# toufique-morshed/CPU-GPU-TFHE

Measured on AMD Instinct MI355X. Metric: gate bootstraps/sec (bootsNAND, N=1024), higher is better.
Workload: dtype f64 (FFT external product; Torus32 in/out, rounded products exact)

## Files before the change

cpu-gpu-tfhe_amd/csrc/keyswitch.hip:

```cpp
#include "engine.h"
#include "modarith.h"

#include <algorithm>
#include <cstdlib>

namespace tfhe_amd {

namespace {


constexpr int kKs4Cols = 4;
constexpr int kKs4Blocks = 126;
constexpr int kKs4I = 32;
#ifndef TFHE_AMD_KS4_THREADS
#define TFHE_AMD_KS4_THREADS 256
#endif
constexpr int kKs4Threads = TFHE_AMD_KS4_THREADS;
constexpr int kKs4ChunkU4 = kKs4I * kKsT * 3;
static_assert(kKs4ChunkU4 % kKs4Threads == 0, "chunk must split evenly");
constexpr int kKs4Pieces = kKs4ChunkU4 / kKs4Threads;

struct KsLane {
    const int32_t *ua, *ua2;
    uint32_t b;
    int32_t *ra, *rb;
};
struct KsPlain {
    const int32_t *u_a, *u_b, *u2_a, *u2_b;
    int32_t add_b;
    int32_t *res_a, *res_b;
    int B;
    __device__ int count() const { return B; }
    __device__ KsLane lane(int ct) const {
        KsLane l;
        l.ua = u_a + (size_t)ct * kN;
        l.ua2 = u2_a ? u2_a + (size_t)ct * kN : nullptr;
        l.b = (uint32_t)u_b[ct] + (uint32_t)add_b + (u2_b ? (uint32_t)u2_b[ct] : 0u);
        l.ra = res_a + (size_t)ct * kn;
        l.rb = res_b + ct;
        return l;
    }
};
struct KsRows {
    const CircKs *ks;
    const int32_t *u_a, *u_b;
    int32_t *wa, *wb;
    int B, nks;
    __device__ int count() const { return B * nks; }
    __device__ KsLane lane(int ct) const {
        const int g = ct / B, k = ct - g * B;
        const CircKs e = ks[g];
        const size_t s1 = (size_t)e.r1 * B + k, so = (size_t)e.out * B + k;
        KsLane l;
        l.ua = u_a + s1 * kN;
        l.b = (uint32_t)u_b[s1] + (uint32_t)e.add_b;
        l.ua2 = nullptr;
        if (e.r2 >= 0) {
            const size_t s2 = (size_t)e.r2 * B + k;
            l.ua2 = u_a + s2 * kN;
            l.b += (uint32_t)u_b[s2];
        }
        l.ra = wa + so * kn;
        l.rb = wb + so;
        return l;
    }
};

template <class P, int SPLIT>
__global__ __launch_bounds__(kKs4Threads) void k_keyswitch_v4(const uint4 *__restrict__ ksk4, P io) {
    __shared__ __attribute__((aligned(16))) uint4 buf[2][kKs4I * kKsT * 4];
    const int part = SPLIT > 1 ? (int)(blockIdx.x % SPLIT) : 0;
    const int bid = SPLIT > 1 ? (int)(blockIdx.x / SPLIT) : (int)blockIdx.x;
    const int xcd = bid & 7, k = bid >> 3;
    const int cb = (k & 15) * 8 + xcd;
    const int ctg = k >> 4;
    if (cb >= kKs4Blocks) return;
    const int tid = threadIdx.x;
    const int ct = ctg * kKs4Threads + tid;
    const bool valid = ct < io.count();
    const KsLane ln = io.lane(valid ? ct : 0);
    for (int t = tid; t < 2 * kKs4I * kKsT; t += kKs4Threads) buf[t >> 8][(t & 255) * 4] = make_uint4(0, 0, 0, 0);

    uint32_t acc[kKs4Cols];
#pragma unroll
    for (int c = 0; c < kKs4Cols; ++c) acc[c] = 0;
    if (SPLIT == 1 && cb * kKs4Cols <= kn && kn < cb * kKs4Cols + kKs4Cols) acc[kn - cb * kKs4Cols] = ln.b;
    constexpr int kIPart = kN / SPLIT;
    const int ibeg = part * kIPart;

    const uint4 *src = ksk4 + ((size_t)cb * kN + ibeg) * kKsT * 3 + tid;
    const uint4 *pa = reinterpret_cast<const uint4 *>(ln.ua + ibeg);
    const uint4 *pa2 = ln.ua2 ? reinterpret_cast<const uint4 *>(ln.ua2 + ibeg) : nullptr;
    int dst[kKs4Pieces];
    uint4 p[kKs4Pieces];
#pragma unroll
    for (int l = 0; l < kKs4Pieces; ++l) {
        const int t = tid + kKs4Threads * l;
        dst[l] = (t / 3) * 4 + (t - 3 * (t / 3)) + 1;
    }
#pragma unroll
    for (int l = 0; l < kKs4Pieces; ++l) p[l] = src[kKs4Threads * l];
    uint4 av[kKs4I / 4], av2[kKs4I / 4];
#pragma unroll
    for (int v = 0; v < kKs4I / 4; ++v) {
        av[v] = pa[v];
        av2[v] = pa2 ? pa2[v] : make_uint4(0, 0, 0, 0);
    }
#pragma unroll
    for (int l = 0; l < kKs4Pieces; ++l) buf[0][dst[l]] = p[l];
    __syncthreads();
    for (int i0 = 0, b = 0; i0 < kIPart; i0 += kKs4I, b ^= 1) {
        uint32_t a[kKs4I];
#pragma unroll
        for (int v = 0; v < kKs4I / 4; ++v) {
            a[4 * v] = av[v].x + av2[v].x + kKsPrecOffset;
            a[4 * v + 1] = av[v].y + av2[v].y + kKsPrecOffset;
            a[4 * v + 2] = av[v].z + av2[v].z + kKsPrecOffset;
            a[4 * v + 3] = av[v].w + av2[v].w + kKsPrecOffset;
        }
        const bool more = i0 + kKs4I < kIPart;
        if (more) {
            const uint4 *sn = src + (size_t)(i0 + kKs4I) * kKsT * 3;
#pragma unroll
            for (int l = 0; l < kKs4Pieces; ++l) p[l] = sn[kKs4Threads * l];
#pragma unroll
            for (int v = 0; v < kKs4I / 4; ++v) {
                av[v] = pa[(i0 + kKs4I) / 4 + v];
                if (pa2) av2[v] = pa2[(i0 + kKs4I) / 4 + v];
            }
        }
        const uint4 *cur = buf[b];
#pragma unroll
        for (int ii = 0; ii < kKs4I; ++ii) {
            const uint32_t ab = a[ii];
#pragma unroll
            for (int j = 0; j < kKsT; ++j) {
                const uint32_t aij = (ab >> (32 - (j + 1) * kKsBasebit)) & (kKsBase - 1);
                const uint4 r = cur[(ii * kKsT + j) * 4 + (int)aij];
                acc[0] -= r.x; acc[1] -= r.y; acc[2] -= r.z; acc[3] -= r.w;
            }
            asm volatile("" : "+v"(acc[0]), "+v"(acc[1]), "+v"(acc[2]), "+v"(acc[3]));
        }
        if (more) {
            uint4 *nb = buf[b ^ 1];
#pragma unroll
            for (int l = 0; l < kKs4Pieces; ++l) nb[dst[l]] = p[l];
        }
        __syncthreads();
    }
    if (!valid) return;
#pragma unroll
    for (int c = 0; c < kKs4Cols; ++c) {
        const int col = cb * kKs4Cols + c;
        int32_t *dst = col < kn ? ln.ra + col : col == kn ? ln.rb : nullptr;
        if (!dst) continue;
        if (SPLIT > 1) atomicAdd(reinterpret_cast<unsigned int *>(dst), acc[c]);
        else *dst = (int32_t)acc[c];
    }
}

constexpr int kKsSmallChunks = 64;
constexpr int kKsSmallI = kN / kKsSmallChunks;

template <class P>
__global__ __launch_bounds__(512) void k_keyswitch_small_init(P io) {
    const KsLane ln = io.lane(blockIdx.x);
    const int col = threadIdx.x;
    if (col < kn) ln.ra[col] = 0;
    else if (col == kn) *ln.rb = (int32_t)ln.b;
}

#ifndef TFHE_AMD_KS_SMALL_U
#define TFHE_AMD_KS_SMALL_U 2
#endif
constexpr int kKsSmallU = TFHE_AMD_KS_SMALL_U;
template <class P, int U>
__global__ __launch_bounds__(512) void k_keyswitch_small(const int32_t *__restrict__ ksk, P io) {
    const int chunk = blockIdx.x, col = threadIdx.x;
    const KsLane ln = io.lane(blockIdx.y);
    if (col > kn) return;
    const int i0 = chunk * kKsSmallI;
    uint32_t acc = 0;
#pragma unroll U
    for (int ii = 0; ii < kKsSmallI; ++ii) {
        const int i = i0 + ii;
        const uint32_t ab = (uint32_t)ln.ua[i] + (ln.ua2 ? (uint32_t)ln.ua2[i] : 0u) + kKsPrecOffset;
        const int32_t *row = ksk + (size_t)i * kKsT * 3 * kKsRow + col;
#pragma unroll
        for (int j = 0; j < kKsT; ++j) {
            const uint32_t h = (ab >> (32 - (j + 1) * kKsBasebit)) & (kKsBase - 1);
            const uint32_t v = (uint32_t)row[(j * 3 + (int)(h ? h : 1u) - 1) * kKsRow];
            acc -= h ? v : 0u;
        }
    }
    int32_t *dst = col < kn ? ln.ra + col : ln.rb;
    atomicAdd(reinterpret_cast<unsigned int *>(dst), acc);
}

typedef int ks5_v4i __attribute__((ext_vector_type(4)));
typedef int ks5_v16i __attribute__((ext_vector_type(16)));
#ifndef TFHE_AMD_KS5_WAVES
#define TFHE_AMD_KS5_WAVES 8
#endif
constexpr int kKs5Waves = TFHE_AMD_KS5_WAVES;
constexpr int kKs5Threads = 64 * kKs5Waves;
constexpr int kKs5Ch = 16;
constexpr int kKs5Nb = 64;
constexpr int kKs5Cols = 8 * kKs5Nb;
static_assert(kKs5Cols > kn, "the N-blocks cover every column and b");
constexpr int kKs5ChU4 = kKs5Ch * 64;
static_assert(kKs5ChU4 % kKs5Threads == 0, "chunk must split evenly");
constexpr int kKs5Pieces = kKs5ChU4 / kKs5Threads;
#ifndef TFHE_AMD_KS5_G
#define TFHE_AMD_KS5_G 8
#endif
constexpr int kKs5G = TFHE_AMD_KS5_G;

template <class P, int SPLIT, int MS>
__global__ __launch_bounds__(kKs5Threads) void k_keyswitch_v5(const uint4 *__restrict__ w5, P io) {
    constexpr int kM = 32 * kKs5Waves * MS;
    constexpr int kG = kKs5G / MS;
    static_assert(kKs5Ch % kG == 0, "groups split the chunk");
    __shared__ __attribute__((aligned(16))) uint2 lut[16][32];
    __shared__ __attribute__((aligned(16))) uint4 bs[2][kKs5Ch][64];
    __shared__ __attribute__((aligned(16))) uint8_t dg[2][2][kM][kKs5Ch];
    const int bid = (int)blockIdx.x, xcd = bid & 7, kk = bid >> 3;
    const int nb = xcd + 8 * (kk & 7), part = (kk >> 3) % SPLIT, mt = (kk >> 3) / SPLIT;
    constexpr int kChunks = kN / kKs5Ch / SPLIT;
    const int c0 = part * kChunks;
    const int tid = threadIdx.x, wave = tid >> 6, l = tid & 63, r = l & 31, hh = l >> 5;
    for (int e = tid; e < 16 * 32; e += kKs5Threads)
        lut[e >> 5][e & 31] = make_uint2(1u << (8 * ((e >> 7) & 3)), 1u << (8 * ((e >> 5) & 3)));
    constexpr int kPer = kKs5Ch * MS / 2;
    constexpr int kU4 = kPer / 4;
    static_assert(kKs5Threads * kPer == kM * kKs5Ch, "loader mapping");
    const int lct = (tid * MS) >> 1, lpart = MS == 1 ? (tid & 1) : 0;
    const int lg = mt * kM + lct;
    const KsLane lln = io.lane(lg < io.count() ? lg : 0);
    const uint4 *pa = reinterpret_cast<const uint4 *>(lln.ua) + kU4 * lpart;
    const uint4 *pa2 = reinterpret_cast<const uint4 *>(lln.ua2 ? lln.ua2 : lln.ua) + kU4 * lpart;
    const uint32_t m2 = lln.ua2 ? 0xffffffffu : 0u;
    pa += c0 * (kKs5Ch / 4);
    pa2 += c0 * (kKs5Ch / 4);
    uint4 uu[kU4], vv[kU4];
#pragma unroll
    for (int q = 0; q < kU4; ++q) {
        uu[q] = pa[q];
        vv[q] = pa2[q];
    }
    auto put_digits = [&](int buf) {
        uint32_t hi[kPer / 4], lo[kPer / 4];
#pragma unroll
        for (int q = 0; q < kU4; ++q) {
            const uint32_t w[4] = {uu[q].x + (vv[q].x & m2) + kKsPrecOffset, uu[q].y + (vv[q].y & m2) + kKsPrecOffset,
                                   uu[q].z + (vv[q].z & m2) + kKsPrecOffset, uu[q].w + (vv[q].w & m2) + kKsPrecOffset};
            hi[q] = (w[0] >> 24) | ((w[1] >> 24) << 8) | ((w[2] >> 24) << 16) | ((w[3] >> 24) << 24);
            lo[q] = ((w[0] >> 16) & 255u) | (((w[1] >> 16) & 255u) << 8) | (((w[2] >> 16) & 255u) << 16) |
                    (((w[3] >> 16) & 255u) << 24);
        }
        if (kU4 == 2) {
            *reinterpret_cast<uint2 *>(&dg[buf][0][lct][kPer * lpart]) = make_uint2(hi[0], hi[1]);
            *reinterpret_cast<uint2 *>(&dg[buf][1][lct][kPer * lpart]) = make_uint2(lo[0], lo[1]);
        } else {
            *reinterpret_cast<uint4 *>(&dg[buf][0][lct][0]) = make_uint4(hi[0], hi[1], hi[2 % kU4], hi[3 % kU4]);
            *reinterpret_cast<uint4 *>(&dg[buf][1][lct][0]) = make_uint4(lo[0], lo[1], lo[2 % kU4], lo[3 % kU4]);
        }
    };
    const uint4 *src = w5 + ((size_t)nb * kN + (size_t)c0 * kKs5Ch) * 64 + tid;
    uint4 p[kKs5Pieces];
#pragma unroll
    for (int q = 0; q < kKs5Pieces; ++q) p[q] = src[q * kKs5Threads];
#pragma unroll
    for (int q = 0; q < kKs5Pieces; ++q) (&bs[0][0][0])[tid + q * kKs5Threads] = p[q];
    put_digits(0);
    __syncthreads();
    ks5_v16i acc[MS];
#pragma unroll
    for (int m = 0; m < MS; ++m) acc[m] = ks5_v16i{};
    for (int c = 0; c < kChunks; ++c) {
        const bool more = c + 1 < kChunks;
        {
            const int cn = more ? c + 1 : c;
            const uint4 *sn = src + (size_t)cn * kKs5ChU4;
#pragma unroll
            for (int q = 0; q < kKs5Pieces; ++q) p[q] = sn[q * kKs5Threads];
#pragma unroll
            for (int q = 0; q < kU4; ++q) {
                uu[q] = pa[cn * (kKs5Ch / 4) + q];
                vv[q] = pa2[cn * (kKs5Ch / 4) + q];
            }
        }
        uint32_t xw[MS][4];
#pragma unroll
        for (int m = 0; m < MS; ++m) {
            const uint4 xd = *reinterpret_cast<const uint4 *>(&dg[c & 1][hh][wave * 32 * MS + 32 * m + r][0]);
            xw[m][0] = xd.x; xw[m][1] = xd.y; xw[m][2] = xd.z; xw[m][3] = xd.w;
        }
        const uint4(*cur)[64] = bs[c & 1];
#pragma unroll
        for (int g = 0; g < kKs5Ch; g += kG) {
            uint4 av[MS][kG], bv[kG];
#pragma unroll
            for (int q = 0; q < kG; ++q) {
                const int ii = g + q;
#pragma unroll
                for (int m = 0; m < MS; ++m) {
                    const uint32_t xb = xw[m][ii >> 2] >> (8 * (ii & 3));
                    const uint2 d01 = lut[(xb >> 4) & 15u][r], d23 = lut[xb & 15u][r];
                    av[m][q] = make_uint4(d01.x, d01.y, d23.x, d23.y);
                }
                bv[q] = cur[ii][l];
            }
            __builtin_amdgcn_sched_barrier(0);
#pragma unroll
            for (int q = 0; q < kG; ++q) {
                const ks5_v4i b = {(int)bv[q].x, (int)bv[q].y, (int)bv[q].z, (int)bv[q].w};
#pragma unroll
                for (int m = 0; m < MS; ++m) {
                    const ks5_v4i a = {(int)av[m][q].x, (int)av[m][q].y, (int)av[m][q].z, (int)av[m][q].w};
                    acc[m] = __builtin_amdgcn_mfma_i32_32x32x32_i8(a, b, acc[m], 0, 0, 0);
                }
            }
        }
        if (more) {
#pragma unroll
            for (int q = 0; q < kKs5Pieces; ++q) (&bs[(c + 1) & 1][0][0])[tid + q * kKs5Threads] = p[q];
            put_digits((c + 1) & 1);
        }
        __syncthreads();
    }
    const int col = nb * 8 + (r >> 2);
    const uint32_t lsh = 8u * (uint32_t)(l & 3);
#pragma unroll
    for (int m = 0; m < MS; ++m) {
#pragma unroll
        for (int reg = 0; reg < 16; ++reg) {
            uint32_t v = (uint32_t)acc[m][reg] << lsh;
            v += (uint32_t)__shfl_xor((int)v, 1, 64);
            v += (uint32_t)__shfl_xor((int)v, 2, 64);
            const int ctm = mt * kM + wave * 32 * MS + 32 * m + (reg & 3) + 8 * (reg >> 2) + 4 * hh;
            if ((l & 3) == 0 && ctm < io.count() && col <= kn) {
                const KsLane lm = io.lane(ctm);
                if (SPLIT > 1) atomicAdd(reinterpret_cast<unsigned int *>(col < kn ? lm.ra + col : lm.rb), 0u - v);
                else if (col < kn) lm.ra[col] = (int32_t)(0u - v);
                else *lm.rb = (int32_t)(lm.b - v);
            }
        }
    }
}

__global__ __launch_bounds__(256) void k_ksk_to_v5(const int32_t *__restrict__ ksk, uint4 *__restrict__ w5) {
    const size_t total = (size_t)kKs5Nb * kN * 64;
    for (size_t t = (size_t)blockIdx.x * 256 + threadIdx.x; t < total; t += (size_t)gridDim.x * 256) {
        const int l = (int)(t & 63);
        const int i = (int)((t >> 6) % kN);
        const int nb = (int)(t / ((size_t)kN * 64));
        const int col = nb * 8 + ((l & 31) >> 2), limb = l & 3, h = l >> 5;
        uint32_t w[4];
#pragma unroll
        for (int tt = 0; tt < 4; ++tt) {
            uint32_t word = 0;
            for (int hh = 1; hh < 4; ++hh) {
                if (col > kn) break;
                uint32_t v = (uint32_t)ksk[(((size_t)i * kKsT + 4 * h + tt) * 3 + (hh - 1)) * kKsRow + col];
                int8_t sb = 0;
                for (int b = 0; b <= limb; ++b) {
                    sb = (int8_t)(v & 0xffu);
                    v = (v - (uint32_t)(int32_t)sb) >> 8;
                }
                word |= (uint32_t)(uint8_t)sb << (8 * hh);
            }
            w[tt] = word;
        }
        w5[t] = make_uint4(w[0], w[1], w[2], w[3]);
    }
}

__global__ __launch_bounds__(256) void k_ksk_to_v4(const int32_t *__restrict__ ksk, uint4 *__restrict__ ksk4) {
    const size_t pieces = (size_t)kKs4Blocks * kN * kKsT * 3;
    for (size_t t = (size_t)blockIdx.x * 256 + threadIdx.x; t < pieces; t += (size_t)gridDim.x * 256) {
        const int cb = (int)(t / ((size_t)kN * kKsT * 3));
        const size_t row = t % ((size_t)kN * kKsT * 3);
        ksk4[t] = *reinterpret_cast<const uint4 *>(ksk + row * kKsRow + cb * kKs4Cols);
    }
}

}

static int ks_split_max() { return 768; }
bool ks5_enabled() {
    static const bool v = [] {
        const char *e = getenv("TFHE_AMD_KS5");
        return !(e && atoi(e) == 0);
    }();
    return v;
}
static int ks5_split(int mtiles) {
    int sp = 1;
    while (sp < 8 && mtiles * kKs5Nb * sp < 512) sp *= 2;
    return sp;
}
template <class P, int MS>
static void launch_ks5(const uint4 *w5, int count, const P &io, hipStream_t s) {
    const int mtiles = (count + 32 * kKs5Waves * MS - 1) / (32 * kKs5Waves * MS);
    const int split = ks5_split(mtiles);
    if (split > 1) hipLaunchKernelGGL(k_keyswitch_small_init<P>, dim3(count), dim3(512), 0, s, io);
    const dim3 grid(mtiles * kKs5Nb * split);
    trace_kernel(split == 8 ? "k_keyswitch_v5(int8-mfma+split8)" : split == 4 ? "k_keyswitch_v5(int8-mfma+split4)"
                 : split == 2 ? "k_keyswitch_v5(int8-mfma+split2)" : "k_keyswitch_v5(int8-mfma)");
    switch (split) {
    case 8: hipLaunchKernelGGL((k_keyswitch_v5<P, 8, MS>), grid, dim3(kKs5Threads), 0, s, w5, io); break;
    case 4: hipLaunchKernelGGL((k_keyswitch_v5<P, 4, MS>), grid, dim3(kKs5Threads), 0, s, w5, io); break;
    case 2: hipLaunchKernelGGL((k_keyswitch_v5<P, 2, MS>), grid, dim3(kKs5Threads), 0, s, w5, io); break;
    default: hipLaunchKernelGGL((k_keyswitch_v5<P, 1, MS>), grid, dim3(kKs5Threads), 0, s, w5, io); break;
    }
}
template <class P>
static void launch_ks4(const DeviceKey &key, int groups, int count, const P &io, hipStream_t s) {
    if (key.ksk5) {
        const uint4 *w5 = reinterpret_cast<const uint4 *>(key.ksk5);
        launch_ks5<P, 1>(w5, count, io, s);
        return;
    }
    trace_kernel("k_keyswitch_v4");
    if (count <= ks_split_max()) {
        hipLaunchKernelGGL(k_keyswitch_small_init<P>, dim3(count), dim3(512), 0, s, io);
        hipLaunchKernelGGL((k_keyswitch_v4<P, 2>), dim3(2 * 128 * groups), dim3(kKs4Threads), 0, s,
                           reinterpret_cast<const uint4 *>(key.ksk4), io);
    } else {
        hipLaunchKernelGGL((k_keyswitch_v4<P, 1>), dim3(128 * groups), dim3(kKs4Threads), 0, s,
                           reinterpret_cast<const uint4 *>(key.ksk4), io);
    }
}

static int ks_unroll_max() { return 4; }

static int ks_small_max() { return ks5_enabled() ? 12 : 96; }

hipError_t launch_keyswitch_rows(const DeviceKey &key, int B, int nks, const CircKs *ks, const int32_t *u_a,
                                 const int32_t *u_b, int32_t *wa, int32_t *wb, hipStream_t s) {
    if (B <= 0 || nks <= 0) return hipSuccess;
    KsRows io{ks, u_a, u_b, wa, wb, B, nks};
    if ((long)B * nks <= ks_small_max()) {
        trace_kernel("k_keyswitch_small");
        hipLaunchKernelGGL(k_keyswitch_small_init<KsRows>, dim3(B * nks), dim3(512), 0, s, io);
        if ((long)B * nks <= ks_unroll_max())
            hipLaunchKernelGGL((k_keyswitch_small<KsRows, kKsSmallI>), dim3(kKsSmallChunks, B * nks), dim3(512), 0, s,
                               key.ksk, io);
        else
            hipLaunchKernelGGL((k_keyswitch_small<KsRows, kKsSmallU>), dim3(kKsSmallChunks, B * nks), dim3(512), 0, s,
                               key.ksk, io);
        return hipGetLastError();
    }
    const int groups = (int)(((size_t)B * nks + kKs4Threads - 1) / kKs4Threads);
    launch_ks4(key, groups, B * nks, io, s);
    return hipGetLastError();
}

__global__ __launch_bounds__(256) void k_circuit_linear(int B, int nlin, const CircLin *__restrict__ lin,
                                                        int32_t *__restrict__ wa, int32_t *__restrict__ wb) {
    const size_t total = (size_t)nlin * B * (kn + 1);
    for (size_t t = (size_t)blockIdx.x * 256 + threadIdx.x; t < total; t += (size_t)gridDim.x * 256) {
        const int w = (int)(t % (kn + 1));
        const size_t gk = t / (kn + 1);
        const int g = (int)(gk / B), k = (int)(gk - (size_t)g * B);
        const CircLin e = lin[g];
        const size_t so = (size_t)e.out * B + k, si = (size_t)(e.in < 0 ? 0 : e.in) * B + k;
        if (w < kn) wa[so * kn + w] = e.in < 0 ? 0 : (int32_t)((uint32_t)e.s * (uint32_t)wa[si * kn + w]);
        else wb[so] = (int32_t)((uint32_t)e.c + (e.in < 0 ? 0u : (uint32_t)e.s * (uint32_t)wb[si]));
    }
}

size_t ksk_v4_words() { return (size_t)kKs4Blocks * kN * kKsT * 3 * 4; }
size_t ksk_v5_words() { return (size_t)kKs5Nb * kN * 64 * 4; }

hipError_t launch_ksk_to_v5(const int32_t *d_ksk, int32_t *d_ksk5, hipStream_t s) {
    hipLaunchKernelGGL(k_ksk_to_v5, dim3(4096), dim3(256), 0, s, d_ksk, reinterpret_cast<uint4 *>(d_ksk5));
    return hipGetLastError();
}

__device__ __forceinline__ double ks_var_one(const int32_t *__restrict__ u, const int32_t *__restrict__ u2,
                                             const double *__restrict__ var) {
    static_assert(kKsT * kKsBasebit == 16 && kKsBase == 4, "digit count below assumes 8 base-4 digits");
    if (var[kKsVarUniform] != 0.0) {
        int k = 0;
#pragma unroll 8
        for (int i = 0; i < kN; ++i) {
            const uint32_t x = ((uint32_t)u[i] + (u2 ? (uint32_t)u2[i] : 0u) + kKsPrecOffset) >> 16;
            k += __builtin_popcount((x | (x >> 1)) & 0x5555u);
        }
        return var[kKsVarUniform + 1 + k];
    }
    double v = 0.0;
    constexpr int U = 4;
    for (int i0 = 0; i0 < kN; i0 += U) {
        uint32_t ab[U];
#pragma unroll
        for (int k = 0; k < U; ++k) ab[k] = (uint32_t)u[i0 + k] + (u2 ? (uint32_t)u2[i0 + k] : 0u) + kKsPrecOffset;
        double t[U][kKsT];
#pragma unroll
        for (int k = 0; k < U; ++k)
#pragma unroll
            for (int j = 0; j < kKsT; ++j) {
                const uint32_t aij = (ab[k] >> (32 - (j + 1) * kKsBasebit)) & (uint32_t)(kKsBase - 1);
                t[k][j] = var[((i0 + k) * kKsT + j) * kKsBase + aij];
            }
#pragma unroll
        for (int k = 0; k < U; ++k)
#pragma unroll
            for (int j = 0; j < kKsT; ++j) {
                const uint32_t aij = (ab[k] >> (32 - (j + 1) * kKsBasebit)) & (uint32_t)(kKsBase - 1);
                v = __dadd_rn(v, aij ? t[k][j] : 0.0);
            }
    }
    return v;
}

__global__ __launch_bounds__(64) void k_ks_variance(const int32_t *__restrict__ u_a, int B, int halves,
                                                    const double *__restrict__ var, double *__restrict__ out) {
    const int g = blockIdx.x * blockDim.x + threadIdx.x;
    if (g >= B) return;
    out[g] = ks_var_one(u_a + (size_t)g * kN, halves == 2 ? u_a + ((size_t)B + g) * kN : nullptr, var);
}

__global__ __launch_bounds__(64) void k_ks_variance_rows(const int32_t *__restrict__ u_a, int B,
                                                         const CircKs *__restrict__ ks, const double *__restrict__ var,
                                                         double *__restrict__ out) {
    const int g = blockIdx.x * blockDim.x + threadIdx.x;
    if (g >= B) return;
    const CircKs k = ks[g];
    out[g] = ks_var_one(u_a + (size_t)k.r1 * kN, k.r2 >= 0 ? u_a + (size_t)k.r2 * kN : nullptr, var);
}

hipError_t launch_ks_variance_rows(const int32_t *u_a, int B, const CircKs *ks, const double *var, double *out,
                                   hipStream_t s) {
    if (B <= 0) return hipSuccess;
    hipLaunchKernelGGL(k_ks_variance_rows, dim3((B + 63) / 64), dim3(64), 0, s, u_a, B, ks, var, out);
    return hipGetLastError();
}

hipError_t launch_ks_variance(const int32_t *u_a, int B, int halves, const double *var, double *out, hipStream_t s) {
    if (B <= 0) return hipSuccess;
    hipLaunchKernelGGL(k_ks_variance, dim3((B + 63) / 64), dim3(64), 0, s, u_a, B, halves, var, out);
    return hipGetLastError();
}

hipError_t launch_circuit_linear(int B, int nlin, const CircLin *lin, int32_t *wa, int32_t *wb, hipStream_t s) {
    if (B <= 0 || nlin <= 0) return hipSuccess;
    const size_t total = (size_t)nlin * B * (kn + 1);
    const int blocks = (int)std::min<size_t>((total + 255) / 256, 65536);
    trace_kernel("k_circuit_linear");
    hipLaunchKernelGGL(k_circuit_linear, dim3(blocks), dim3(256), 0, s, B, nlin, lin, wa, wb);
    return hipGetLastError();
}

hipError_t launch_ksk_to_v4(const int32_t *d_ksk, int32_t *d_ksk4, hipStream_t s) {
    hipLaunchKernelGGL(k_ksk_to_v4, dim3(2048), dim3(256), 0, s, d_ksk, reinterpret_cast<uint4 *>(d_ksk4));
    return hipGetLastError();
}

int ks_version() { return ks5_enabled() ? 5 : 4; }

hipError_t launch_keyswitch(const DeviceKey &key, int B, const int32_t *u_a, const int32_t *u_b,
                            const int32_t *u2_a, const int32_t *u2_b, int32_t add_b,
                            int32_t *res_a, int32_t *res_b, hipStream_t s) {
    if (B <= 0) return hipSuccess;
    if (B <= ks_small_max()) {
        trace_kernel("k_keyswitch_small");
        KsPlain io{u_a, u_b, u2_a, u2_b, add_b, res_a, res_b, B};
        hipLaunchKernelGGL(k_keyswitch_small_init<KsPlain>, dim3(B), dim3(512), 0, s, io);
        if (B <= ks_unroll_max())
            hipLaunchKernelGGL((k_keyswitch_small<KsPlain, kKsSmallI>), dim3(kKsSmallChunks, B), dim3(512), 0, s,
                               key.ksk, io);
        else
            hipLaunchKernelGGL((k_keyswitch_small<KsPlain, kKsSmallU>), dim3(kKsSmallChunks, B), dim3(512), 0, s,
                               key.ksk, io);
    } else {
        const int groups = (B + kKs4Threads - 1) / kKs4Threads;
        KsPlain io{u_a, u_b, u2_a, u2_b, add_b, res_a, res_b, B};
        launch_ks4(key, groups, B, io, s);
    }
    return hipGetLastError();
}

}
```

Measured before the change: 332,000.

## Pack keyswitch int8 MFMA K-dimension densely, dropping zero digit slots

Before this change, each MFMA K slice held 4 key digits times 4 byte slots, and one slot per digit was always zero (hh=0 unused), so a quarter of the K work and of the key bytes was padding. The key is now repacked so that 16 input quads fill 3 dense MFMA K slices, and the one-hot A operands are assembled from two shifted LUT halves. This is meant to cut MFMA count and key-weight bandwidth by about a quarter. In exchange it drops the MS multi-tile template, changes the default group size, and adds a uint2 tail load path plus a more intricate key conversion.

```diff
diff --git a/cpu-gpu-tfhe_amd/csrc/keyswitch.hip b/cpu-gpu-tfhe_amd/csrc/keyswitch.hip
--- a/cpu-gpu-tfhe_amd/csrc/keyswitch.hip
+++ b/cpu-gpu-tfhe_amd/csrc/keyswitch.hip
@@ -204,38 +204,50 @@
 #endif
 constexpr int kKs5Waves = TFHE_AMD_KS5_WAVES;
 constexpr int kKs5Threads = 64 * kKs5Waves;
-constexpr int kKs5Ch = 16;
+constexpr int kKs5M = 32 * kKs5Waves;
+#ifndef TFHE_AMD_KS5_CH
+#define TFHE_AMD_KS5_CH 16
+#endif
+constexpr int kKs5Ch = TFHE_AMD_KS5_CH;
+static_assert(kKs5Ch == 16 || kKs5Ch == 32, "digit rows of one or two uint4");
+constexpr int kKs5Quads = kKs5Ch / 4;
 constexpr int kKs5Nb = 64;
 constexpr int kKs5Cols = 8 * kKs5Nb;
 static_assert(kKs5Cols > kn, "the N-blocks cover every column and b");
-constexpr int kKs5ChU4 = kKs5Ch * 64;
-static_assert(kKs5ChU4 % kKs5Threads == 0, "chunk must split evenly");
+constexpr int kKs5QuadU4 = 3 * 64;
+constexpr int kKs5ChU4 = kKs5Quads * kKs5QuadU4;
 constexpr int kKs5Pieces = kKs5ChU4 / kKs5Threads;
+constexpr bool kKs5Half = kKs5ChU4 % kKs5Threads != 0;
+static_assert(kKs5ChU4 % kKs5Threads == (kKs5Half ? kKs5Threads / 2 : 0), "chunk splits into uint4 + uint2 pieces");
 #ifndef TFHE_AMD_KS5_G
-#define TFHE_AMD_KS5_G 8
+#define TFHE_AMD_KS5_G 4
 #endif
 constexpr int kKs5G = TFHE_AMD_KS5_G;
-
-template <class P, int SPLIT, int MS>
+static_assert(kKs5G % 4 == 0 && kKs5Quads % (kKs5G / 4) == 0, "read groups are whole quads and split the chunk");
+
+__host__ __device__ constexpr uint32_t ks5_onehot(uint32_t a) { return (1u << (8 * a)) >> 8; }
+
+template <class P, int SPLIT>
 __global__ __launch_bounds__(kKs5Threads) void k_keyswitch_v5(const uint4 *__restrict__ w5, P io) {
-    constexpr int kM = 32 * kKs5Waves * MS;
-    constexpr int kG = kKs5G / MS;
-    static_assert(kKs5Ch % kG == 0, "groups split the chunk");
-    __shared__ __attribute__((aligned(16))) uint2 lut[16][32];
-    __shared__ __attribute__((aligned(16))) uint4 bs[2][kKs5Ch][64];
-    __shared__ __attribute__((aligned(16))) uint8_t dg[2][2][kM][kKs5Ch];
+    constexpr int kQ = kKs5G / 4;
+    __shared__ __attribute__((aligned(16))) uint2 lut[2][16][32];
+    __shared__ __attribute__((aligned(16))) uint4 bs[2][3 * kKs5Quads][64];
+    __shared__ __attribute__((aligned(16))) uint8_t dg[2][2][kKs5M][kKs5Ch];
     const int bid = (int)blockIdx.x, xcd = bid & 7, kk = bid >> 3;
     const int nb = xcd + 8 * (kk & 7), part = (kk >> 3) % SPLIT, mt = (kk >> 3) / SPLIT;
     constexpr int kChunks = kN / kKs5Ch / SPLIT;
     const int c0 = part * kChunks;
     const int tid = threadIdx.x, wave = tid >> 6, l = tid & 63, r = l & 31, hh = l >> 5;
-    for (int e = tid; e < 16 * 32; e += kKs5Threads)
-        lut[e >> 5][e & 31] = make_uint2(1u << (8 * ((e >> 7) & 3)), 1u << (8 * ((e >> 5) & 3)));
-    constexpr int kPer = kKs5Ch * MS / 2;
+    for (int e = tid; e < 2 * 16 * 32; e += kKs5Threads) {
+        const uint64_t six = (uint64_t)ks5_onehot((e >> 7) & 3) | (uint64_t)ks5_onehot((e >> 5) & 3) << 24;
+        const uint64_t v = (e >> 9) ? six << 16 : six;
+        lut[e >> 9][(e >> 5) & 15][e & 31] = make_uint2((uint32_t)v, (uint32_t)(v >> 32));
+    }
+    constexpr int kPer = kKs5Ch / 2;
     constexpr int kU4 = kPer / 4;
-    static_assert(kKs5Threads * kPer == kM * kKs5Ch, "loader mapping");
-    const int lct = (tid * MS) >> 1, lpart = MS == 1 ? (tid & 1) : 0;
-    const int lg = mt * kM + lct;
+    static_assert(kKs5Threads * kPer == kKs5M * kKs5Ch, "loader mapping");
+    const int lct = tid >> 1, lpart = tid & 1;
+    const int lg = mt * kKs5M + lct;
     const KsLane lln = io.lane(lg < io.count() ? lg : 0);
     const uint4 *pa = reinterpret_cast<const uint4 *>(lln.ua) + kU4 * lpart;
     const uint4 *pa2 = reinterpret_cast<const uint4 *>(lln.ua2 ? lln.ua2 : lln.ua) + kU4 * lpart;
@@ -249,7 +261,7 @@
         vv[q] = pa2[q];
     }
     auto put_digits = [&](int buf) {
-        uint32_t hi[kPer / 4], lo[kPer / 4];
+        uint32_t hi[kU4], lo[kU4];
 #pragma unroll
         for (int q = 0; q < kU4; ++q) {
             const uint32_t w[4] = {uu[q].x + (vv[q].x & m2) + kKsPrecOffset, uu[q].y + (vv[q].y & m2) + kKsPrecOffset,
@@ -262,69 +274,80 @@
             *reinterpret_cast<uint2 *>(&dg[buf][0][lct][kPer * lpart]) = make_uint2(hi[0], hi[1]);
             *reinterpret_cast<uint2 *>(&dg[buf][1][lct][kPer * lpart]) = make_uint2(lo[0], lo[1]);
         } else {
-            *reinterpret_cast<uint4 *>(&dg[buf][0][lct][0]) = make_uint4(hi[0], hi[1], hi[2 % kU4], hi[3 % kU4]);
-            *reinterpret_cast<uint4 *>(&dg[buf][1][lct][0]) = make_uint4(lo[0], lo[1], lo[2 % kU4], lo[3 % kU4]);
+            *reinterpret_cast<uint4 *>(&dg[buf][0][lct][kPer * lpart]) = make_uint4(hi[0], hi[1], hi[2 % kU4], hi[3 % kU4]);
+            *reinterpret_cast<uint4 *>(&dg[buf][1][lct][kPer * lpart]) = make_uint4(lo[0], lo[1], lo[2 % kU4], lo[3 % kU4]);
         }
     };
-    const uint4 *src = w5 + ((size_t)nb * kN + (size_t)c0 * kKs5Ch) * 64 + tid;
+    const uint4 *wg = w5 + ((size_t)nb * (kN / 4) + (size_t)c0 * kKs5Quads) * kKs5QuadU4;
+    const uint4 *src = wg + tid;
+    const uint2 *src2 = reinterpret_cast<const uint2 *>(wg + kKs5Pieces * kKs5Threads) + tid;
     uint4 p[kKs5Pieces];
-#pragma unroll
-    for (int q = 0; q < kKs5Pieces; ++q) p[q] = src[q * kKs5Threads];
-#pragma unroll
-    for (int q = 0; q < kKs5Pieces; ++q) (&bs[0][0][0])[tid + q * kKs5Threads] = p[q];
+    uint2 p2 = make_uint2(0, 0);
+    auto fetch = [&](int cn) {
+#pragma unroll
+        for (int q = 0; q < kKs5Pieces; ++q) p[q] = src[(size_t)cn * kKs5ChU4 + q * kKs5Threads];
+        if constexpr (kKs5Half) p2 = src2[(size_t)cn * kKs5ChU4 * 2];
+    };
+    auto stage = [&](int buf) {
+#pragma unroll
+        for (int q = 0; q < kKs5Pieces; ++q) (&bs[buf][0][0])[tid + q * kKs5Threads] = p[q];
+        if constexpr (kKs5Half) reinterpret_cast<uint2 *>(&bs[buf][0][0] + kKs5Pieces * kKs5Threads)[tid] = p2;
+    };
+    fetch(0);
+    stage(0);
     put_digits(0);
     __syncthreads();
-    ks5_v16i acc[MS];
-#pragma unroll
-    for (int m = 0; m < MS; ++m) acc[m] = ks5_v16i{};
+    ks5_v16i acc = ks5_v16i{};
     for (int c = 0; c < kChunks; ++c) {
         const bool more = c + 1 < kChunks;
         {
             const int cn = more ? c + 1 : c;
-            const uint4 *sn = src + (size_t)cn * kKs5ChU4;
-#pragma unroll
-            for (int q = 0; q < kKs5Pieces; ++q) p[q] = sn[q * kKs5Threads];
+            fetch(cn);
 #pragma unroll
             for (int q = 0; q < kU4; ++q) {
                 uu[q] = pa[cn * (kKs5Ch / 4) + q];
                 vv[q] = pa2[cn * (kKs5Ch / 4) + q];
             }
         }
-        uint32_t xw[MS][4];
-#pragma unroll
-        for (int m = 0; m < MS; ++m) {
-            const uint4 xd = *reinterpret_cast<const uint4 *>(&dg[c & 1][hh][wave * 32 * MS + 32 * m + r][0]);
-            xw[m][0] = xd.x; xw[m][1] = xd.y; xw[m][2] = xd.z; xw[m][3] = xd.w;
+        uint32_t xw[kKs5Quads];
+#pragma unroll
+        for (int q = 0; q < kKs5Quads / 4; ++q) {
+            const uint4 xd = *reinterpret_cast<const uint4 *>(&dg[c & 1][hh][wave * 32 + r][16 * q]);
+            xw[4 * q] = xd.x; xw[4 * q + 1] = xd.y; xw[4 * q + 2] = xd.z; xw[4 * q + 3] = xd.w;
         }
         const uint4(*cur)[64] = bs[c & 1];
 #pragma unroll
-        for (int g = 0; g < kKs5Ch; g += kG) {
-            uint4 av[MS][kG], bv[kG];
-#pragma unroll
-            for (int q = 0; q < kG; ++q) {
-                const int ii = g + q;
-#pragma unroll
-                for (int m = 0; m < MS; ++m) {
-                    const uint32_t xb = xw[m][ii >> 2] >> (8 * (ii & 3));
-                    const uint2 d01 = lut[(xb >> 4) & 15u][r], d23 = lut[xb & 15u][r];
-                    av[m][q] = make_uint4(d01.x, d01.y, d23.x, d23.y);
+        for (int g = 0; g < kKs5Quads; g += kQ) {
+            uint2 hv[kQ][4], lv[kQ][4];
+            uint4 bv[kQ][3];
+#pragma unroll
+            for (int q = 0; q < kQ; ++q) {
+#pragma unroll
+                for (int ii = 0; ii < 4; ++ii) {
+                    const uint32_t xb = xw[g + q] >> (8 * ii);
+                    hv[q][ii] = lut[0][(xb >> 4) & 15u][r];
+                    lv[q][ii] = lut[1][xb & 15u][r];
                 }
-                bv[q] = cur[ii][l];
+#pragma unroll
+                for (int s = 0; s < 3; ++s) bv[q][s] = cur[3 * (g + q) + s][l];
             }
             __builtin_amdgcn_sched_barrier(0);
 #pragma unroll
-            for (int q = 0; q < kG; ++q) {
-                const ks5_v4i b = {(int)bv[q].x, (int)bv[q].y, (int)bv[q].z, (int)bv[q].w};
-#pragma unroll
-                for (int m = 0; m < MS; ++m) {
-                    const ks5_v4i a = {(int)av[m][q].x, (int)av[m][q].y, (int)av[m][q].z, (int)av[m][q].w};
-                    acc[m] = __builtin_amdgcn_mfma_i32_32x32x32_i8(a, b, acc[m], 0, 0, 0);
+            for (int q = 0; q < kQ; ++q) {
+                const uint2 *h = hv[q], *lo = lv[q];
+                const ks5_v4i a[3] = {
+                    {(int)h[0].x, (int)(h[0].y | lo[0].x), (int)lo[0].y, (int)h[1].x},
+                    {(int)(h[1].y | lo[1].x), (int)lo[1].y, (int)h[2].x, (int)(h[2].y | lo[2].x)},
+                    {(int)lo[2].y, (int)h[3].x, (int)(h[3].y | lo[3].x), (int)lo[3].y}};
+#pragma unroll
+                for (int s = 0; s < 3; ++s) {
+                    const ks5_v4i b = {(int)bv[q][s].x, (int)bv[q][s].y, (int)bv[q][s].z, (int)bv[q][s].w};
+                    acc = __builtin_amdgcn_mfma_i32_32x32x32_i8(a[s], b, acc, 0, 0, 0);
                 }
             }
         }
         if (more) {
-#pragma unroll
-            for (int q = 0; q < kKs5Pieces; ++q) (&bs[(c + 1) & 1][0][0])[tid + q * kKs5Threads] = p[q];
+            stage((c + 1) & 1);
             put_digits((c + 1) & 1);
         }
         __syncthreads();
@@ -332,45 +355,39 @@
     const int col = nb * 8 + (r >> 2);
     const uint32_t lsh = 8u * (uint32_t)(l & 3);
 #pragma unroll
-    for (int m = 0; m < MS; ++m) {
-#pragma unroll
-        for (int reg = 0; reg < 16; ++reg) {
-            uint32_t v = (uint32_t)acc[m][reg] << lsh;
-            v += (uint32_t)__shfl_xor((int)v, 1, 64);
-            v += (uint32_t)__shfl_xor((int)v, 2, 64);
-            const int ctm = mt * kM + wave * 32 * MS + 32 * m + (reg & 3) + 8 * (reg >> 2) + 4 * hh;
-            if ((l & 3) == 0 && ctm < io.count() && col <= kn) {
-                const KsLane lm = io.lane(ctm);
-                if (SPLIT > 1) atomicAdd(reinterpret_cast<unsigned int *>(col < kn ? lm.ra + col : lm.rb), 0u - v);
-                else if (col < kn) lm.ra[col] = (int32_t)(0u - v);
-                else *lm.rb = (int32_t)(lm.b - v);
-            }
+    for (int reg = 0; reg < 16; ++reg) {
+        uint32_t v = (uint32_t)acc[reg] << lsh;
+        v += (uint32_t)__shfl_xor((int)v, 1, 64);
+        v += (uint32_t)__shfl_xor((int)v, 2, 64);
+        const int ctm = mt * kKs5M + wave * 32 + (reg & 3) + 8 * (reg >> 2) + 4 * hh;
+        if ((l & 3) == 0 && ctm < io.count() && col <= kn) {
+            const KsLane lm = io.lane(ctm);
+            if (SPLIT > 1) atomicAdd(reinterpret_cast<unsigned int *>(col < kn ? lm.ra + col : lm.rb), 0u - v);
+            else if (col < kn) lm.ra[col] = (int32_t)(0u - v);
+            else *lm.rb = (int32_t)(lm.b - v);
         }
     }
 }
 
 __global__ __launch_bounds__(256) void k_ksk_to_v5(const int32_t *__restrict__ ksk, uint4 *__restrict__ w5) {
-    const size_t total = (size_t)kKs5Nb * kN * 64;
+    const size_t total = (size_t)kKs5Nb * (kN / 4) * kKs5QuadU4;
     for (size_t t = (size_t)blockIdx.x * 256 + threadIdx.x; t < total; t += (size_t)gridDim.x * 256) {
         const int l = (int)(t & 63);
-        const int i = (int)((t >> 6) % kN);
-        const int nb = (int)(t / ((size_t)kN * 64));
-        const int col = nb * 8 + ((l & 31) >> 2), limb = l & 3, h = l >> 5;
-        uint32_t w[4];
-#pragma unroll
-        for (int tt = 0; tt < 4; ++tt) {
-            uint32_t word = 0;
-            for (int hh = 1; hh < 4; ++hh) {
-                if (col > kn) break;
-                uint32_t v = (uint32_t)ksk[(((size_t)i * kKsT + 4 * h + tt) * 3 + (hh - 1)) * kKsRow + col];
-                int8_t sb = 0;
-                for (int b = 0; b <= limb; ++b) {
-                    sb = (int8_t)(v & 0xffu);
-                    v = (v - (uint32_t)(int32_t)sb) >> 8;
-                }
-                word |= (uint32_t)(uint8_t)sb << (8 * hh);
-            }
-            w[tt] = word;
+        const int s = (int)((t >> 6) % 3);
+        const int G = (int)((t / kKs5QuadU4) % (kN / 4));
+        const int nb = (int)(t / ((size_t)(kN / 4) * kKs5QuadU4));
+        const int col = nb * 8 + ((l & 31) >> 2), limb = l & 3, hh = l >> 5;
+        uint32_t w[4] = {0, 0, 0, 0};
+        for (int q = 0; q < 16 && col <= kn; ++q) {
+            const int slot = 16 * s + q, e = slot / 3, h1 = slot - 3 * e;
+            const int i = 4 * G + (e >> 2), j = 4 * hh + (e & 3);
+            uint32_t v = (uint32_t)ksk[(((size_t)i * kKsT + j) * 3 + h1) * kKsRow + col];
+            int8_t sb = 0;
+            for (int b = 0; b <= limb; ++b) {
+                sb = (int8_t)(v & 0xffu);
+                v = (v - (uint32_t)(int32_t)sb) >> 8;
+            }
+            w[q >> 2] |= (uint32_t)(uint8_t)sb << (8 * (q & 3));
         }
         w5[t] = make_uint4(w[0], w[1], w[2], w[3]);
     }
@@ -395,31 +412,34 @@
     }();
     return v;
 }
+#ifndef TFHE_AMD_KS5_WGS
+#define TFHE_AMD_KS5_WGS 512
+#endif
 static int ks5_split(int mtiles) {
     int sp = 1;
-    while (sp < 8 && mtiles * kKs5Nb * sp < 512) sp *= 2;
+    while (sp < 8 && mtiles * kKs5Nb * sp < TFHE_AMD_KS5_WGS) sp *= 2;
     return sp;
 }
-template <class P, int MS>
+template <class P>
 static void launch_ks5(const uint4 *w5, int count, const P &io, hipStream_t s) {
-    const int mtiles = (count + 32 * kKs5Waves * MS - 1) / (32 * kKs5Waves * MS);
+    const int mtiles = (count + kKs5M - 1) / kKs5M;
     const int split = ks5_split(mtiles);
     if (split > 1) hipLaunchKernelGGL(k_keyswitch_small_init<P>, dim3(count), dim3(512), 0, s, io);
     const dim3 grid(mtiles * kKs5Nb * split);
     trace_kernel(split == 8 ? "k_keyswitch_v5(int8-mfma+split8)" : split == 4 ? "k_keyswitch_v5(int8-mfma+split4)"
                  : split == 2 ? "k_keyswitch_v5(int8-mfma+split2)" : "k_keyswitch_v5(int8-mfma)");
     switch (split) {
-    case 8: hipLaunchKernelGGL((k_keyswitch_v5<P, 8, MS>), grid, dim3(kKs5Threads), 0, s, w5, io); break;
-    case 4: hipLaunchKernelGGL((k_keyswitch_v5<P, 4, MS>), grid, dim3(kKs5Threads), 0, s, w5, io); break;
-    case 2: hipLaunchKernelGGL((k_keyswitch_v5<P, 2, MS>), grid, dim3(kKs5Threads), 0, s, w5, io); break;
-    default: hipLaunchKernelGGL((k_keyswitch_v5<P, 1, MS>), grid, dim3(kKs5Threads), 0, s, w5, io); break;
+    case 8: hipLaunchKernelGGL((k_keyswitch_v5<P, 8>), grid, dim3(kKs5Threads), 0, s, w5, io); break;
+    case 4: hipLaunchKernelGGL((k_keyswitch_v5<P, 4>), grid, dim3(kKs5Threads), 0, s, w5, io); break;
+    case 2: hipLaunchKernelGGL((k_keyswitch_v5<P, 2>), grid, dim3(kKs5Threads), 0, s, w5, io); break;
+    default: hipLaunchKernelGGL((k_keyswitch_v5<P, 1>), grid, dim3(kKs5Threads), 0, s, w5, io); break;
     }
 }
 template <class P>
 static void launch_ks4(const DeviceKey &key, int groups, int count, const P &io, hipStream_t s) {
     if (key.ksk5) {
         const uint4 *w5 = reinterpret_cast<const uint4 *>(key.ksk5);
-        launch_ks5<P, 1>(w5, count, io, s);
+        launch_ks5(w5, count, io, s);
         return;
     }
     trace_kernel("k_keyswitch_v4");
@@ -472,7 +492,7 @@
 }
 
 size_t ksk_v4_words() { return (size_t)kKs4Blocks * kN * kKsT * 3 * 4; }
-size_t ksk_v5_words() { return (size_t)kKs5Nb * kN * 64 * 4; }
+size_t ksk_v5_words() { return (size_t)kKs5Nb * (kN / 4) * kKs5QuadU4 * 4; }
 
 hipError_t launch_ksk_to_v5(const int32_t *d_ksk, int32_t *d_ksk5, hipStream_t s) {
     hipLaunchKernelGGL(k_ksk_to_v5, dim3(4096), dim3(256), 0, s, d_ksk, reinterpret_cast<uint4 *>(d_ksk5));
```

Result: no change. 331,000 (-0.3%).
